# bronemos/view-fusion

Measured on AMD Instinct MI355X. Metric: denoise_steps_per_sec, higher is better.
Workload: dtype f32; 1 GPU; small UNet 64x64 (33.9M params), B=16/GPU N=6 (S=96 views/GPU), training iteration fwd+bwd+Adam, linear T=2000 schedule; global_batch=16, views=6, parallelism=dp1, launch=HIP-graph replay of the whole iteration

## Files before the change

view_fusion_amd/csrc/conv.hip:

```cpp
#include "common.h"
#include "wgrad_reduce.h"
#include <cstring>
#include "conv1x1.h"
#include "any_geom.h"
#include <cstdlib>

namespace {

constexpr int TCO = 64;
constexpr int WGRAD_TARGET_WGS = 512;

template <int KS, int LOGW, int MODE, int TPIX = 128>
struct Geo {
    static constexpr int W = 1 << LOGW;
    static constexpr int H = W;
    static constexpr int HW = W * H;
    static constexpr int IM = HW >= TPIX ? 1 : TPIX / HW;
    static constexpr int TH = HW >= TPIX ? TPIX / W : H;
    static constexpr int TPI = HW >= TPIX ? HW / TPIX : 1;
    static constexpr int PAD = KS / 2;
    static constexpr int PH = MODE == 1 ? 2 * TH + 1 : (MODE == 4 ? TH + 1 : TH + 2 * PAD);
    static constexpr int PW = KS == 1 ? W : (MODE == 1 ? 2 * W + 4 : (MODE == 4 ? W + 4 : W + 8));
    static constexpr int CO = (KS == 1 || MODE == 4) ? 0 : 3;
    static constexpr int Q = (MODE == 1 ? 2 * W : W) / 4;
    static constexpr int PS = IM * PH * PW;
    static constexpr int SH = MODE == 1 ? 2 * H : (MODE == 2 ? H / 2 : H);
    static constexpr int SW = MODE == 1 ? 2 * W : (MODE == 2 ? W / 2 : W);
    static __host__ __device__ constexpr int pix_off(int p) {
        const int im = IM > 1 ? (p >> (2 * LOGW)) : 0;
        const int q = p & (HW - 1);
        const int r = IM > 1 ? (q >> LOGW) : (p >> LOGW);
        const int c = p & (W - 1);
        return MODE == 1 ? im * PH * PW + 2 * r * PW + 2 * c + CO : im * PH * PW + r * PW + c + CO;
    }
};

struct ConvArgs {
    const float* x;
    const float* w;
    const float* bias;
    const float* vbias;
    const float* res;
    float* y;
    int S, Cin, Cout, CinP, CoutP;
    int ksplit;
    float* ws;
    const float* x2;
    float* y2;
    int C1, C1o;
    const float* gn_gamma = nullptr;
    const float* gn_beta = nullptr;
    float* gn_out = nullptr;
    float* gn_stats = nullptr;
    int gn_groups = 0, gn_silu = 0, gn_store_y = 1;
    float gn_eps = 1e-5f;
};

template <class G, int MODE, bool SAFE = false>
__device__ __forceinline__ float4 load_patch4(const float* __restrict__ x, int S, int Cin, int s, int ci,
                                              int r0, int pr, int q) {
    float4 v = make_float4(0.f, 0.f, 0.f, 0.f);
    if (SAFE && MODE == 0 && G::PAD == 0)
        return *reinterpret_cast<const float4*>(x + ((size_t)s * Cin + ci) * (size_t)(G::SH * G::SW) + (r0 + pr) * G::SW + 4 * q);
    if (s >= S || ci >= Cin) return v;
    const size_t plane = ((size_t)s * Cin + ci) * (size_t)(G::SH * G::SW);
    if (MODE == 0) {
        const int gy = r0 + pr - G::PAD;
        if (gy >= 0 && gy < G::H) v = *reinterpret_cast<const float4*>(x + plane + gy * G::SW + 4 * q);
    } else if (MODE == 1) {
        const int gy = 2 * r0 + pr - 1;
        if (gy >= 0 && gy < G::SH) v = *reinterpret_cast<const float4*>(x + plane + gy * G::SW + 4 * q);
    } else if (MODE == 4) {
        const int gy = r0 + pr;
        if (gy < G::H) v = *reinterpret_cast<const float4*>(x + plane + gy * G::SW + 4 * q);
    } else {
        const int uy = r0 + pr - G::PAD;
        if (uy >= 0 && uy < G::H) {
            const float2 t = *reinterpret_cast<const float2*>(x + plane + (uy >> 1) * G::SW + 2 * q);
            v = make_float4(t.x, t.x, t.y, t.y);
        }
    }
    return v;
}

template <int KS, int LOGW, int MODE, int NPT, int NCO = 1, bool SAFE = false>
__global__ __launch_bounds__(256, (KS == 1 && NPT == 1 && NCO == 1) ? 5 : 1) void conv_mfma_kernel(ConvArgs a) {
    constexpr int TPIX = 64 * NPT;
    using G = Geo<KS, LOGW, MODE, TPIX>;
    constexpr int CK = KS == 3 ? 8 : 32;
    constexpr int NG = KS == 3 ? 9 : 4;
    constexpr int WROW = 12;
    constexpr int NW4 = NG * TCO * 2;
    constexpr int NX4 = CK * G::IM * G::PH * G::Q;

    constexpr int WLS = NG * TCO * WROW;
    __shared__ __attribute__((aligned(16))) float wl[NCO * WLS];
    __shared__ __attribute__((aligned(16))) float xl[CK * G::PS];

    const int tid = threadIdx.x, lane = tid & 63, wid = tid >> 6;
    const int cw = wid & 1, pw = wid >> 1;
    const int li = lane & 31, lh = lane >> 5;

    const int ncot1 = a.CoutP / TCO;
    const int ncot = (ncot1 + NCO - 1) / NCO;
    const unsigned logical0 = xcd_remap(blockIdx.x, gridDim.x);
    const int split = logical0 % a.ksplit;
    const unsigned logical = logical0 / a.ksplit;
    const int cot = logical % ncot;
    const int tile = logical / ncot;
    const int co0 = cot * NCO * TCO;
    const int nco_here = min(NCO, ncot1 - cot * NCO);
    const int nch = a.CinP / CK;
    const int cbeg = (split * nch / a.ksplit) * CK, cend = ((split + 1) * nch / a.ksplit) * CK;
    const int s0 = G::IM > 1 ? tile * G::IM : tile / G::TPI;
    const int r0 = G::IM > 1 ? 0 : (tile % G::TPI) * G::TH;

#ifdef VF_CONV_STAMPS
    long long st_[4] = {clock64(), 0, 0, 0}, rt_[2] = {wall_clock64(), 0};
#endif
    if (KS != 1)
        for (int i = tid; i < CK * G::PS; i += 256) xl[i] = 0.f;

    constexpr int NWF = NW4 / 256, NXF = NX4 / 256;
    constexpr bool WT = (NW4 % 256) != 0, XT = (NX4 % 256) != 0;
    static_assert(NCO == 1 || !WT, "multi-tile workgroups assume whole 256-wide weight passes");
    constexpr int PD = 1;
    float4 wreg[PD][NCO * (NWF > 0 ? NWF : 1)], xreg[PD][NXF > 0 ? NXF : 1];
    float4 wtail[PD], xtail[PD];
#pragma unroll
    for (int d = 0; d < PD; ++d) wtail[d] = xtail[d] = make_float4(0.f, 0.f, 0.f, 0.f);
    const size_t wtile = (size_t)(a.CinP / CK) * (NG * TCO * 8);
    const float* wsrc = a.w + (size_t)cot * NCO * wtile;
    auto load_w = [&](int e, int c0, int j = 0) -> float4 {
        return *reinterpret_cast<const float4*>(wsrc + (size_t)min(j, nco_here - 1) * wtile +
                                                (size_t)(c0 / CK) * (NG * TCO * 8) + 4 * e);
    };
    auto load_x = [&](int e, int c0) -> float4 {
        const int q = e % G::Q;
        const int t1 = e / G::Q;
        const int pr = t1 % G::PH;
        const int t2 = t1 / G::PH;
        const int im = t2 % G::IM, ci = t2 / G::IM;
        if (KS == 1 && a.x2) {
            const bool second = c0 >= a.C1;
            return load_patch4<G, MODE, SAFE>(second ? a.x2 : a.x, a.S, second ? a.Cin - a.C1 : a.C1, s0 + im,
                                              second ? c0 - a.C1 + ci : c0 + ci, r0, pr, q);
        }
        return load_patch4<G, MODE, SAFE>(a.x, a.S, a.Cin, s0 + im, c0 + ci, r0, pr, q);
    };
    auto store_x = [&](int e, const float4& v) {
        const int q = e % G::Q;
        const int t1 = e / G::Q;
        *reinterpret_cast<float4*>(xl + t1 * G::PW + 4 * q + ((KS == 1 || MODE == 4) ? 0 : 4)) = v;
    };
#define VF_LOAD_CHUNK(D_, C0)                                                         \
    {                                                                                 \
// ... 247 lines not shown

    f32x16 acc[NT];
#pragma unroll
    for (int t = 0; t < NT; ++t) acc[t] = (f32x16){0};

    const float* ab = dyl + (cw * 32 + li) * DYS + kq * 64 + 4 * lh;
    const float* bb = xl + (ciw * 32 + li) * PSO + G::pix_off(kq * 64 + 4 * lh);

    constexpr int NXF = NX4 / 256;
    constexpr bool XT = (NX4 % 256) != 0;
    constexpr bool PF = BIG;
    float4 dreg[ND4 / 256], xreg[NXF > 0 ? NXF : 1];
    float4 xtail = make_float4(0.f, 0.f, 0.f, 0.f);
    auto load_dy = [&](int e, int tile) -> float4 {
        const int s0 = G::IM > 1 ? tile * G::IM : tile / G::TPI;
        const int r0 = G::IM > 1 ? 0 : (tile % G::TPI) * G::TH;
        const int q = e & 31, co = e >> 5;
        const int p = 4 * q;
        const int s = G::IM > 1 ? s0 + (p >> (2 * LOGW)) : s0;
        const int pix = G::IM > 1 ? (p & (OHW - 1)) : r0 * G::W + p;
        float4 v = make_float4(0.f, 0.f, 0.f, 0.f);
        if (s < a.S && co0 + co < a.Cout)
            v = *reinterpret_cast<const float4*>(a.dy + ((size_t)s * a.Cout + co0 + co) * OHW + pix);
        return v;
    };
    auto load_x = [&](int e, int tile) -> float4 {
        const int s0 = G::IM > 1 ? tile * G::IM : tile / G::TPI;
        const int r0 = G::IM > 1 ? 0 : (tile % G::TPI) * G::TH;
        const int q = e % G::Q;
        const int t1 = e / G::Q;
        const int pr = t1 % G::PH;
        const int t2 = t1 / G::PH;
        const int im = t2 % G::IM, ci = t2 / G::IM;
        if (KS == 1 && a.x2) {
            const bool second = ci0 >= a.C1;
            return load_patch4<G, MODE>(second ? a.x2 : a.x, a.S, second ? a.Cin - a.C1 : a.C1, s0 + im,
                                        second ? ci0 - a.C1 + ci : ci0 + ci, r0, pr, q);
        }
        return load_patch4<G, MODE>(a.x, a.S, a.Cin, s0 + im, ci0 + ci, r0, pr, q);
    };
    auto store_x = [&](int e, const float4& v) {
        const int q = e % G::Q;
        const int t1 = e / G::Q;
        const int ci = t1 / (G::IM * G::PH), rest = t1 % (G::IM * G::PH);
        float* d = xl + ci * PSO + rest * G::PW + 4 * q + (KS == 1 ? 0 : 4);
        d[0] = v.x; d[1] = v.y; d[2] = v.z; d[3] = v.w;
    };
#define VF_WG_LOAD(TILE)                                                                    \
    {                                                                                       \
        _Pragma("unroll") for (int i = 0; i < ND4 / 256; ++i) dreg[i] = load_dy(tid + i * 256, (TILE)); \
        _Pragma("unroll") for (int i = 0; i < NXF; ++i) xreg[i] = load_x(tid + i * 256, (TILE));        \
        if (XT && tid + NXF * 256 < NX4) xtail = load_x(tid + NXF * 256, (TILE));            \
    }
#define VF_WG_STORE()                                                                       \
    {                                                                                       \
        _Pragma("unroll") for (int i = 0; i < ND4 / 256; ++i) {                              \
            const int e = tid + i * 256;                                                    \
            *reinterpret_cast<float4*>(dyl + (e >> 5) * DYS + 4 * (e & 31)) = dreg[i];       \
        }                                                                                   \
        _Pragma("unroll") for (int i = 0; i < NXF; ++i) store_x(tid + i * 256, xreg[i]);     \
        if (XT && tid + NXF * 256 < NX4) store_x(tid + NXF * 256, xtail);                    \
    }

    if (PF && t_begin < t_end) VF_WG_LOAD(t_begin);
    for (int tile = t_begin; tile < t_end; ++tile) {
        __syncthreads();
        if (!PF) VF_WG_LOAD(tile);
        VF_WG_STORE();
        __syncthreads();
        if (PF && tile + 1 < t_end) VF_WG_LOAD(tile + 1);
        constexpr int NSTG = (BIG ? 16 : 8) * KS;
        auto frag_b = [&](int stg, int kw, int e) -> float {
            const int grp = stg / KS, kh = stg % KS;
            const int d = G::pix_off(8 * grp) - G::pix_off(0);
            return bb[d + (MODE == 1 ? 2 * e : e) + kh * G::PW + kw];
        };
        float b_cur[KS][4];
#pragma unroll
        for (int kw = 0; kw < KS; ++kw)
#pragma unroll
            for (int e = 0; e < 4; ++e) b_cur[kw][e] = frag_b(0, kw, e);
        float4 a4 = *reinterpret_cast<const float4*>(ab);
#pragma unroll
        for (int stg = 0; stg < NSTG; ++stg) {
            float b_nxt[KS][4];
            float4 a_nxt = a4;
            if (stg + 1 < NSTG) {
#pragma unroll
                for (int kw = 0; kw < KS; ++kw)
#pragma unroll
                    for (int e = 0; e < 4; ++e) b_nxt[kw][e] = frag_b(stg + 1, kw, e);
                if ((stg + 1) % KS == 0) a_nxt = *reinterpret_cast<const float4*>(ab + 8 * ((stg + 1) / KS));
            }
            __builtin_amdgcn_sched_barrier(0);
            const float av[4] = {a4.x, a4.y, a4.z, a4.w};
#pragma unroll
            for (int e = 0; e < 4; ++e)
#pragma unroll
                for (int kw = 0; kw < KS; ++kw) {
                    const int tap = (stg % KS) * KS + kw;
                    acc[tap] = __builtin_amdgcn_mfma_f32_32x32x2f32(av[e], b_cur[kw][e], acc[tap], 0, 0, 0);
                }
            __builtin_amdgcn_sched_barrier(0);
            if (stg + 1 < NSTG) {
                a4 = a_nxt;
#pragma unroll
                for (int kw = 0; kw < KS; ++kw)
#pragma unroll
                    for (int e = 0; e < 4; ++e) b_cur[kw][e] = b_nxt[kw][e];
            }
        }
    }

#undef VF_WG_LOAD
#undef VF_WG_STORE
    constexpr int NTP = NT > 1 ? (NT + 1) / 2 : 1;
    static_assert(2 * NTP * 16 * 64 <= LDSF, "k-half reduce buffer does not fit");
#pragma unroll
    for (int t0 = 0; t0 < (BIG ? 0 : NT); t0 += NTP) {
        __syncthreads();
        if (kq == 1) {
#pragma unroll
            for (int t = t0; t < (t0 + NTP < NT ? t0 + NTP : NT); ++t)
#pragma unroll
                for (int r = 0; r < 16; ++r) lds[((cw * NTP + (t - t0)) * 16 + r) * 64 + lane] = acc[t][r];
        }
        __syncthreads();
        if (kq == 0) {
#pragma unroll
            for (int t = t0; t < (t0 + NTP < NT ? t0 + NTP : NT); ++t)
#pragma unroll
                for (int r = 0; r < 16; ++r) acc[t][r] += lds[((cw * NTP + (t - t0)) * 16 + r) * 64 + lane];
        }
    }
    if (kq != 0) return;
    const int slab = bz;
#pragma unroll
    for (int tap = 0; tap < NT; ++tap) {
#pragma unroll
        for (int r = 0; r < 16; ++r) {
            const int co = co0 + cw * 32 + (r & 3) + 8 * (r >> 2) + 4 * lh;
            const int ci = ci0 + ciw * 32 + li;
            if (ci < a.CinQ) a.ws[(((size_t)slab * NT + tap) * a.CoutP + co) * a.CinQ + ci] = acc[tap][r];
        }
    }
}

__global__ __launch_bounds__(256) void wgrad_reduce_kernel(const float* __restrict__ ws, float* __restrict__ dw,
                                                           int nslab, int NT, int Cout, int Cin, int CoutP,
                                                           int CinQ) {
    wgrad_reduce_body(ws, dw, nslab, NT, Cout, Cin, CoutP, CinQ, (int)blockIdx.x);
}

struct Wgrad1Args {
    const float* x;
    const float* x2;
    const float* dy;
    float* ws;
    int S, Cin, Cout, CoutP, CinQ, C1, HW;
    int nsteps, steps_per_slice;
};

template <int TM, int TN>
__global__ __launch_bounds__(256, 2) void conv1x1_wgrad_kernel(Wgrad1Args a) {
    constexpr int KP = 64, RS = KP + 4;
    constexpr int NI = TM / 64, NJ = TN / 64;
    constexpr int ND = TM * 16 / 256, NX = TN * 16 / 256;
    __shared__ __attribute__((aligned(16))) float Dl[TM * RS];
    __shared__ __attribute__((aligned(16))) float Xl[TN * RS];
    const int tid = threadIdx.x, lane = tid & 63, wid = tid >> 6;
    const int cw = wid & 1, ciw = wid >> 1, li = lane & 31, lh = lane >> 5;
    const unsigned lgc = xcd_remap(blockIdx.x + gridDim.x * (blockIdx.y + gridDim.y * blockIdx.z),
                                   gridDim.x * gridDim.y * gridDim.z);
    const int bx = lgc % gridDim.x, by = (lgc / gridDim.x) % gridDim.y, bz = lgc / (gridDim.x * gridDim.y);
    const int co0 = bx * TM, ci0 = by * TN;
    const int t_begin = bz * a.steps_per_slice;
    const int t_end = min(a.nsteps, t_begin + a.steps_per_slice);
    const int spv = a.HW / KP;

    const int srow = tid >> 4, sq = tid & 15;
    size_t doff[8], xoff[8];
    const float* xb[8];
#pragma unroll
    for (int i = 0; i < 8; ++i) {
        const int row = srow + 16 * i;
        doff[i] = (size_t)min(co0 + row, a.Cout - 1) * a.HW + 4 * sq;
        const int ci = min(ci0 + row, a.Cin - 1);
        const bool second = a.x2 && ci >= a.C1;
        xb[i] = second ? a.x2 : a.x;
        xoff[i] = (size_t)(second ? ci - a.C1 : ci) * a.HW + 4 * sq;
    }
    const int xC = a.x2 ? a.C1 : a.Cin, x2C = a.Cin - a.C1;
    float4 dr0, dr1, dr2, dr3, dr4, dr5, dr6, dr7, xr0, xr1, xr2, xr3, xr4, xr5, xr6, xr7;
    dr0 = dr1 = dr2 = dr3 = dr4 = dr5 = dr6 = dr7 = xr0 = xr1 = xr2 = xr3 = xr4 = xr5 = xr6 = xr7 =
        make_float4(0.f, 0.f, 0.f, 0.f);
#define VF_W1_LD(I, T_)                                                                                   \
    {                                                                                                     \
        const int sv = (T_) / spv, p0 = ((T_) % spv) * KP;                                                 \
        if constexpr ((I) < ND)                                                                           \
            dr##I = *reinterpret_cast<const float4*>(a.dy + (size_t)sv * a.Cout * a.HW + doff[I] + p0);    \
        if constexpr ((I) < NX)                                                                           \
            xr##I = *reinterpret_cast<const float4*>(xb[I] + (size_t)sv * (xb[I] == a.x ? xC : x2C) * a.HW + xoff[I] + p0); \
    }
#define VF_W1_ST(I)                                                                                       \
    {                                                                                                     \
        if constexpr ((I) < ND) *reinterpret_cast<float4*>(Dl + (srow + 16 * (I)) * RS + 4 * sq) = dr##I;   \
        if constexpr ((I) < NX) *reinterpret_cast<float4*>(Xl + (srow + 16 * (I)) * RS + 4 * sq) = xr##I;   \
    }
#define VF_W1_LOAD(T_) { VF_W1_LD(0, T_) VF_W1_LD(1, T_) VF_W1_LD(2, T_) VF_W1_LD(3, T_) VF_W1_LD(4, T_) VF_W1_LD(5, T_) VF_W1_LD(6, T_) VF_W1_LD(7, T_) }
#define VF_W1_STORE() { VF_W1_ST(0) VF_W1_ST(1) VF_W1_ST(2) VF_W1_ST(3) VF_W1_ST(4) VF_W1_ST(5) VF_W1_ST(6) VF_W1_ST(7) }

    f32x16 acc[NI][NJ];
#pragma unroll
    for (int i = 0; i < NI; ++i)
#pragma unroll
        for (int j = 0; j < NJ; ++j) acc[i][j] = (f32x16){0};
    const float* ab = Dl + (cw * (TM / 2) + li) * RS + 4 * lh;
    const float* bb = Xl + (ciw * (TN / 2) + li) * RS + 4 * lh;

    if (t_begin < t_end) {
        VF_W1_LOAD(t_begin);
        for (int t = t_begin; t < t_end; ++t) {
            __syncthreads();
            VF_W1_STORE();
            __syncthreads();
            VF_W1_LOAD(min(t + 1, t_end - 1));
            float4 fa[NI], fb[NJ];
#pragma unroll
            for (int i = 0; i < NI; ++i) fa[i] = *reinterpret_cast<const float4*>(ab + 32 * i * RS);
#pragma unroll
            for (int j = 0; j < NJ; ++j) fb[j] = *reinterpret_cast<const float4*>(bb + 32 * j * RS);
#pragma unroll
            for (int g = 0; g < KP / 8; ++g) {
                float4 na[NI], nb[NJ];
#pragma unroll
                for (int i = 0; i < NI; ++i) na[i] = fa[i];
#pragma unroll
                for (int j = 0; j < NJ; ++j) nb[j] = fb[j];
                if (g + 1 < KP / 8) {
#pragma unroll
                    for (int i = 0; i < NI; ++i) na[i] = *reinterpret_cast<const float4*>(ab + 32 * i * RS + 8 * (g + 1));
#pragma unroll
                    for (int j = 0; j < NJ; ++j) nb[j] = *reinterpret_cast<const float4*>(bb + 32 * j * RS + 8 * (g + 1));
                }
                __builtin_amdgcn_sched_barrier(0);
#pragma unroll
                for (int i = 0; i < NI; ++i)
#pragma unroll
                    for (int j = 0; j < NJ; ++j) {
                        acc[i][j] = __builtin_amdgcn_mfma_f32_32x32x2f32(fa[i].x, fb[j].x, acc[i][j], 0, 0, 0);
                        acc[i][j] = __builtin_amdgcn_mfma_f32_32x32x2f32(fa[i].y, fb[j].y, acc[i][j], 0, 0, 0);
                        acc[i][j] = __builtin_amdgcn_mfma_f32_32x32x2f32(fa[i].z, fb[j].z, acc[i][j], 0, 0, 0);
                        acc[i][j] = __builtin_amdgcn_mfma_f32_32x32x2f32(fa[i].w, fb[j].w, acc[i][j], 0, 0, 0);
                    }
                __builtin_amdgcn_sched_barrier(0);
#pragma unroll
                for (int i = 0; i < NI; ++i) fa[i] = na[i];
#pragma unroll
                for (int j = 0; j < NJ; ++j) fb[j] = nb[j];
            }
        }
    }
#undef VF_W1_LD
#undef VF_W1_ST
#undef VF_W1_LOAD
#undef VF_W1_STORE
    float* sb = a.ws + (size_t)bz * a.CoutP * a.CinQ;
#pragma unroll
    for (int i = 0; i < NI; ++i)
#pragma unroll
        for (int j = 0; j < NJ; ++j) {
            const int ci = ci0 + ciw * (TN / 2) + j * 32 + li;
#pragma unroll
            for (int r = 0; r < 16; ++r) {
                const int co = co0 + cw * (TM / 2) + i * 32 + (r & 3) + 8 * (r >> 2) + 4 * lh;
                sb[(size_t)co * a.CinQ + ci] = acc[i][j][r];
            }
        }
}

__device__ __forceinline__ void pack_one(const float* __restrict__ w, float* __restrict__ wf,
                                         float* __restrict__ wb, int Cout, int Cin, int KS, size_t nf, size_t nb,
                                         size_t idx) {
    const int NT = KS * KS, CK = KS == 3 ? 8 : 32, NG = KS == 3 ? 9 : 4;
    const bool bwd = idx >= nf;
    if (bwd) {
        idx -= nf;
        if (idx >= nb || !wb) return;
    }
    const int M = bwd ? Cin : Cout, K = bwd ? Cout : Cin;
    const int nchunk = (K + CK - 1) / CK;
    const int k8 = idx & 7;
    const int m = (idx >> 3) & 63;
    size_t t = idx >> 9;
    const int g = t % NG;
    t /= NG;
    const int chunk = t % nchunk;
    const int mt = t / nchunk;
    const int mm = mt * 64 + m;
    const int kk = chunk * CK + (KS == 3 ? k8 : g * 8 + k8);
    const int tap = KS == 3 ? (bwd ? NT - 1 - g : g) : 0;
    float v = 0.f;
    if (mm < M && kk < K) {
        const int co = bwd ? kk : mm, ci = bwd ? mm : kk;
        v = w[((size_t)co * Cin + ci) * NT + tap];
    }
    (bwd ? wb : wf)[idx] = v;
}

__global__ void pack_weights_kernel(const float* __restrict__ w, float* __restrict__ wf, float* __restrict__ wb,
                                    int Cout, int Cin, int KS, size_t nf, size_t nb) {
    pack_one(w, wf, wb, Cout, Cin, KS, nf, nb, (size_t)blockIdx.x * blockDim.x + threadIdx.x);
}

struct PackDesc {
    const float* w;
    float* wf;
    float* wb;
    long long Cout, Cin, KS, nf, nb, first_block;
};
__global__ void pack_weights_multi_kernel(const PackDesc* __restrict__ desc, int nlayers) {
    int lo = 0, hi = nlayers;
    while (hi - lo > 1) {
        const int mid = (lo + hi) >> 1;
        if (desc[mid].first_block <= (long long)blockIdx.x) lo = mid; else hi = mid;
    }
    const PackDesc d = desc[lo];
    const size_t idx = ((size_t)blockIdx.x - (size_t)d.first_block) * blockDim.x + threadIdx.x;
    pack_one(d.w, d.wf, d.wb, (int)d.Cout, (int)d.Cin, (int)d.KS, (size_t)d.nf, (size_t)d.nb, idx);
}

__global__ void sumpool2_kernel(const float* __restrict__ x, float* __restrict__ y, size_t n_out, int Wo) {
    const size_t i = (size_t)blockIdx.x * blockDim.x + threadIdx.x;
    if (i >= n_out) return;
    const size_t row = i / Wo;
    const int w = i - row * Wo;
    const float* p = x + row * 2 * (2 * Wo) + 2 * w;
    y[i] = (p[0] + p[1]) + (p[2 * Wo] + p[2 * Wo + 1]);
}

__global__ void conv_splitk_reduce_kernel(const float4* __restrict__ ws, const float* __restrict__ bias,
                                          const float* __restrict__ vbias, const float4* __restrict__ res,
                                          float4* __restrict__ y, int ksplit, size_t n4, int HW4, int Cout) {
    const size_t i = (size_t)blockIdx.x * blockDim.x + threadIdx.x;
    if (i >= n4) return;
    const size_t sc = i / HW4;
    float b = 0.f;
    if (bias) b += bias[sc % Cout];
    if (vbias) b += vbias[sc];
    float4 r = make_float4(0.f, 0.f, 0.f, 0.f);
    if (res) r = res[i];
    float4 v = make_float4(0.f, 0.f, 0.f, 0.f);
    for (int k0 = 0; k0 < ksplit; k0 += 8) {
        float4 t[8];
#pragma unroll
        for (int j = 0; j < 8; ++j) t[j] = ws[(size_t)min(k0 + j, ksplit - 1) * n4 + i];
#pragma unroll
        for (int j = 0; j < 8; ++j) {
            if (k0 + j < ksplit) { v.x += t[j].x; v.y += t[j].y; v.z += t[j].z; v.w += t[j].w; }
        }
    }
    y[i] = make_float4(v.x + r.x + b, v.y + r.y + b, v.z + r.z + b, v.w + r.w + b);
}

template <int NV, int NT>
__global__ __launch_bounds__(NT) void conv_splitk_reduce_gn_kernel(const float4* __restrict__ ws, const float* __restrict__ bias,
                                                                    const float* __restrict__ vbias,
                                                                    const float4* __restrict__ res, float4* __restrict__ y,
                                                                    const float* __restrict__ gamma,
                                                                    const float* __restrict__ beta, float4* __restrict__ a_out,
                                                                    int ksplit, size_t n4_total, int hw4sh, int Cout, int cpg,
                                                                    float eps, int silu) {
    __shared__ float red[NT / 64];
    constexpr int KB = NV >= 8 ? 1 : 8 / NV;
    const int G = Cout / cpg;
    const int sg = blockIdx.x, s = sg / G, g = sg - s * G;
    const int n4 = cpg << hw4sh;
    const size_t base4 = ((size_t)s * Cout + (size_t)g * cpg) << hw4sh;
    float4 v[NV];
    size_t gi[NV];
#pragma unroll
    for (int i = 0; i < NV; ++i) {
        v[i] = make_float4(0.f, 0.f, 0.f, 0.f);
        gi[i] = base4 + min((int)threadIdx.x + i * NT, n4 - 1);
    }
    for (int k0 = 0; k0 < ksplit; k0 += KB) {
        float4 t[KB][NV];
#pragma unroll
        for (int kk = 0; kk < KB; ++kk)
#pragma unroll
            for (int i = 0; i < NV; ++i) t[kk][i] = ws[(size_t)min(k0 + kk, ksplit - 1) * n4_total + gi[i]];
#pragma unroll
        for (int kk = 0; kk < KB; ++kk)
            if (k0 + kk < ksplit) {
#pragma unroll
                for (int i = 0; i < NV; ++i) { v[i].x += t[kk][i].x; v[i].y += t[kk][i].y; v[i].z += t[kk][i].z; v[i].w += t[kk][i].w; }
            }
    }
    float gam[NV], bet[NV];
    float sum = 0.f;
#pragma unroll
    for (int i = 0; i < NV; ++i) {
        const int idx = min((int)threadIdx.x + i * NT, n4 - 1);
        const int c = g * cpg + (idx >> hw4sh);
        float b = 0.f;
        if (bias) b += bias[c];
        if (vbias) b += vbias[(size_t)s * Cout + c];
        float4 r = make_float4(0.f, 0.f, 0.f, 0.f);
        if (res) r = res[gi[i]];
        v[i] = make_float4(v[i].x + r.x + b, v[i].y + r.y + b, v[i].z + r.z + b, v[i].w + r.w + b);
        gam[i] = gamma[c];
        bet[i] = beta[c];
        const bool ok = (int)threadIdx.x + i * NT < n4;
        if (y && ok) y[gi[i]] = v[i];
        if (!ok) v[i] = make_float4(0.f, 0.f, 0.f, 0.f);
        sum += (v[i].x + v[i].y) + (v[i].z + v[i].w);
    }
    const float inv_n = 1.0f / (float)(n4 * 4);
    const float mean = block_sum<NT>(sum, red) * inv_n;
    float sq = 0.f;
#pragma unroll
    for (int i = 0; i < NV; ++i) {
        const float a = v[i].x - mean, b = v[i].y - mean, c = v[i].z - mean, d = v[i].w - mean;
        const float q = (a * a + b * b) + (c * c + d * d);
        sq += (int)threadIdx.x + i * NT < n4 ? q : 0.f;
    }
    const float var = block_sum<NT>(sq, red) * inv_n;
    const float rstd = 1.0f / sqrtf(var + eps);
#pragma unroll
    for (int i = 0; i < NV; ++i) {
        if ((int)threadIdx.x + i * NT < n4) {
            const float ga = gam[i] * rstd;
// ... 238 lines not shown
    hipLaunchKernelGGL(pack_weights_kernel, dim3((unsigned)((n + 255) / 256)), dim3(256), 0, (hipStream_t)stream,
                       w_oihw, w_fwd, w_bwd, Cout, Cin, KS, nf, nb);
    VF_RETURN_LAST_ERROR();
}

int vf_conv_pack_weights_multi(const void* desc, int nlayers, long total_blocks, void* stream) {
    if (nlayers <= 0 || total_blocks <= 0) return 0;
    hipLaunchKernelGGL(pack_weights_multi_kernel, dim3((unsigned)total_blocks), dim3(256), 0, (hipStream_t)stream,
                       (const PackDesc*)desc, nlayers);
    VF_RETURN_LAST_ERROR();
}

struct GnFuse {
    const float* gamma;
    const float* beta;
    float* out;
    float* stats;
    int groups, silu, store_y;
    float eps;
};

static int conv_fwd_impl(const float* x, const float* x2, int C1, const float* w_packed, const float* bias,
                         const float* view_bias, const float* residual, float* y, float* y2, int C1o, float* ws,
                         long ws_floats, int S, int Cin, int Cout, int H, int W, int KS, int mode, void* stream,
                         const GnFuse* gn = nullptr) {
    if (S <= 0) return 0;
    const int lw = ilog2_exact(W);
    if (!conv_fwd_args_ok(Cin, Cout, KS, mode, x2 != nullptr, C1, y2 != nullptr, C1o, gn != nullptr, gn ? gn->groups : 0))
        return (int)hipErrorInvalidValue;
    const ConvFwdPlan p = conv_fwd_plan(S, Cin, Cout, H, W, KS, mode, x2 != nullptr, C1, y2 != nullptr, C1o, gn != nullptr,
                                        gn ? gn->groups : 0, ws != nullptr, ws_floats);
    if (p.route == ROUTE_ANY) {
        const int e = vfi_conv_any_fwd(x, x2, C1, w_packed, bias, view_bias, residual, y, y2, C1o, ws, ws_floats, S, Cin, Cout,
                                       H, W, KS, mode, (hipStream_t)stream);
        if (e || !gn) return e;
        return vf_gn_fwd(y, gn->gamma, gn->beta, gn->out, gn->stats, gn->stats + (size_t)S * gn->groups, S, Cout, H * W,
                         gn->groups, gn->eps, gn->silu, stream);
    }
    ConvArgs a;
    a.x = x; a.w = w_packed; a.bias = bias; a.vbias = view_bias; a.res = residual; a.y = y;
    a.x2 = x2; a.C1 = C1; a.y2 = y2; a.C1o = C1o;
    if (y2) ws = nullptr;
    a.S = S; a.Cin = Cin; a.Cout = Cout;
    a.CinP = round_up(Cin, KS == 3 ? 8 : 32);
    a.CoutP = round_up(Cout, TCO);
    a.ksplit = 1;
    a.ws = ws;
    if (gn) {
        a.gn_gamma = gn->gamma; a.gn_beta = gn->beta; a.gn_out = gn->out; a.gn_stats = gn->stats;
        a.gn_groups = gn->groups; a.gn_silu = gn->silu; a.gn_store_y = gn->store_y; a.gn_eps = gn->eps;
    }
    hipStream_t st = (hipStream_t)stream;
    if (p.route == ROUTE_1X1_64 || p.route == ROUTE_1X1_128) {
        C11Args c = conv1x1_shape(S, Cin, Cout, H, W, C1, C1o);
        c.x = x; c.x2 = x2; c.w = w_packed; c.bias = bias; c.vbias = view_bias; c.res = residual; c.y = y; c.y2 = y2;
        return vfi_conv1x1_launch(c, st);
    }
#define VF_CASE(KS_, LW_, M_) \
    if (KS == KS_ && lw == LW_ && mode == M_) return launch_conv<KS_, LW_, M_>(a, st, p);
    VF_CASE(3, 3, 0) VF_CASE(3, 4, 0) VF_CASE(3, 5, 0) VF_CASE(3, 6, 0) VF_CASE(3, 7, 0)
    VF_CASE(3, 3, 1) VF_CASE(3, 4, 1) VF_CASE(3, 5, 1) VF_CASE(3, 6, 1)
    VF_CASE(3, 4, 2) VF_CASE(3, 5, 2) VF_CASE(3, 6, 2) VF_CASE(3, 7, 2)
    VF_CASE(3, 3, 4) VF_CASE(3, 4, 4) VF_CASE(3, 5, 4) VF_CASE(3, 6, 4)
    VF_CASE(1, 3, 0) VF_CASE(1, 4, 0) VF_CASE(1, 5, 0) VF_CASE(1, 6, 0) VF_CASE(1, 7, 0)
#undef VF_CASE
    return (int)hipErrorInvalidValue;
}

int vf_conv_fwd(const float* x, const float* w_packed, const float* bias, const float* view_bias,
                const float* residual, float* y, float* ws, long ws_floats, int S, int Cin, int Cout, int H,
                int W, int KS, int mode, void* stream) {
    return conv_fwd_impl(x, nullptr, Cin, w_packed, bias, view_bias, residual, y, nullptr, Cout, ws, ws_floats, S, Cin,
                         Cout, H, W, KS, mode, stream);
}

int vf_conv_fwd_gn(const float* x, const float* w_packed, const float* bias, const float* view_bias, const float* residual,
                   float* y, int store_y, const float* gn_gamma, const float* gn_beta, float* a_out, float* gn_stats,
                   int groups, float eps, int silu, float* ws, long ws_floats, int S, int Cin, int Cout, int H, int W,
                   int KS, int mode, void* stream) {
    GnFuse gn{gn_gamma, gn_beta, a_out, gn_stats, groups, silu, store_y, eps};
    return conv_fwd_impl(x, nullptr, Cin, w_packed, bias, view_bias, residual, y, nullptr, Cout, ws, ws_floats, S, Cin,
                         Cout, H, W, KS, mode, stream, &gn);
}

int vf_conv1x1_cat_fwd(const float* x1, const float* x2, int C1, const float* w_packed, const float* bias, float* y,
                       float* ws, long ws_floats, int S, int Cin, int Cout, int H, int W, void* stream) {
    return conv_fwd_impl(x1, x2, C1, w_packed, bias, nullptr, nullptr, y, nullptr, Cout, ws, ws_floats, S, Cin, Cout, H, W,
                         1, 0, stream);
}

int vf_conv1x1_cat_dgrad(const float* dy, const float* w_packed_bwd, float* dx1, float* dx2, int C1, int S, int Cin,
                         int Cout, int H, int W, void* stream) {
    return conv_fwd_impl(dy, nullptr, Cout, w_packed_bwd, nullptr, nullptr, nullptr, dx1, dx2, C1, nullptr, 0, S, Cout, Cin,
                         H, W, 1, 0, stream);
}

long vf_conv_fwd_ws_floats(int S, int Cin, int Cout, int H, int W, int KS) {
    if (!square_pow2(H, W)) return vfi_conv_any_fwd_ws_floats(S, Cin, Cout, H, W, KS);
    const long tiles64 = ((long)S * H * W + 63) / 64;
    const long nblk_min = ((long)S * H * W + 127) / 128 * (round_up(Cout, TCO) / TCO);
    (void)tiles64;
    const int nch = round_up(Cin, KS == 3 ? 8 : 32) / (KS == 3 ? 8 : 32);
    const int ks = choose_ksplit((int)nblk_min, nch);
    return ks > 1 ? (long)ks * S * Cout * H * W : 0;
}

int vf_conv_fwd_plan(int S, int Cin, int Cout, int H, int W, int KS, int mode, int C1, int C1o, int gn_groups, int has_ws,
                     long ws_floats, int* out) {
    if (!out || S <= 0 || Cin <= 0 || Cout <= 0 || H <= 0 || W <= 0) return (int)hipErrorInvalidValue;
    const bool cat = C1 > 0 && C1 < Cin, split = C1o > 0 && C1o < Cout, gn = gn_groups > 0;
    if (!conv_fwd_args_ok(Cin, Cout, KS, mode, cat, C1, split, C1o, gn, gn_groups)) return (int)hipErrorInvalidValue;
    if (mode != 0 && mode != 1 && mode != 2 && mode != 4) return (int)hipErrorInvalidValue;
    if (!fwd_specialised(KS, H, W, mode) && mode == 2 && ((H & 1) || (W & 1))) return (int)hipErrorInvalidValue;
    const ConvFwdPlan p = conv_fwd_plan(S, Cin, Cout, H, W, KS, mode, cat, C1, split, C1o, gn, gn_groups, has_ws != 0,
                                        ws_floats);
    const int v[8] = {p.route, p.npt, p.nblk, p.ks, p.safe, p.reduce, p.nv, p.nt};
    memcpy(out, v, sizeof v);
    return 0;
}

long vf_conv_wgrad_ws_floats(int S, int Cin, int Cout, int H, int W, int KS) {
    if (!square_pow2(H, W)) return vfi_conv_any_wgrad_ws_floats(S, Cin, Cout, H, W, KS);
    if (KS == 1) {
        const int tm = wgrad1_tile(Cout), tn = wgrad1_tile(Cin);
        const long slab1 = (long)round_up(Cout, tm) * round_up(Cin, tn);
        long z1 = WGRAD_TARGET_WGS / ((round_up(Cout, tm) / tm) * (round_up(Cin, tn) / tn));
        const long nsteps = (long)S * (H * W / 64);
        if (z1 > nsteps / 4) z1 = nsteps / 4;
        if (z1 < 1) z1 = 1;
        return z1 * slab1;
    }
    const long slab = (long)KS * KS * round_up(Cout, TCO) * round_up(Cin, 32);
    const int nco = round_up(Cout, TCO) / TCO, nci = round_up(Cin, 32) / 32;
    long z = (WGRAD_TARGET_WGS + nco * nci - 1) / (nco * nci);
    long ntiles = ((long)S * H * W + 127) / 128;
    if (z > ntiles) z = ntiles;
    if (z < 1) z = 1;
    return z * slab;
}

static int conv_wgrad_impl(const float* x, const float* x2, int C1, const float* dy, float* dw, float* ws,
                           long ws_floats, int S, int Cin, int Cout, int H, int W, int KS, int mode, void* stream,
                           long long* desc = nullptr, int* nblocks = nullptr) {
    if (desc) *nblocks = 0;
    if (S <= 0) return 0;
    const int lw = ilog2_exact(W);
    if (KS != 1 && KS != 3) return (int)hipErrorInvalidValue;
    if (KS == 1 && mode != 0) return (int)hipErrorInvalidValue;
    if (x2 && (KS != 1 || C1 <= 0 || C1 >= Cin || C1 % 64 != 0)) return (int)hipErrorInvalidValue;
    if (!wgrad_specialised(KS, H, W, mode))
        return vfi_conv_any_wgrad(x, x2, C1, dy, dw, ws, ws_floats, S, Cin, Cout, H, W, KS, mode, (hipStream_t)stream, desc,
                                  nblocks);
    if (KS == 1) {
        Wgrad1Args g;
        g.x = x; g.x2 = x2; g.dy = dy; g.ws = ws; g.S = S; g.Cin = Cin; g.Cout = Cout; g.C1 = C1; g.HW = H * W;
        const int tm = wgrad1_tile(Cout), tn = wgrad1_tile(Cin);
        g.CoutP = round_up(Cout, tm); g.CinQ = round_up(Cin, tn);
        g.nsteps = S * (H * W / 64);
        const int nco = g.CoutP / tm, nci = g.CinQ / tn;
        const size_t slab = (size_t)g.CoutP * g.CinQ;
        int z = WGRAD_TARGET_WGS / (nco * nci);
        if (z > g.nsteps / 4) z = g.nsteps / 4;
        if (z < 1) z = 1;
        if ((size_t)ws_floats < slab) return (int)hipErrorInvalidValue;
        if ((size_t)z > (size_t)ws_floats / slab) z = (int)((size_t)ws_floats / slab);
        g.steps_per_slice = (g.nsteps + z - 1) / z;
        z = (g.nsteps + g.steps_per_slice - 1) / g.steps_per_slice;
        hipStream_t st1 = (hipStream_t)stream;
        const dim3 grid(nco, nci, z);
        if (tm == 128 && tn == 128) hipLaunchKernelGGL((conv1x1_wgrad_kernel<128, 128>), grid, dim3(256), 0, st1, g);
        else if (tm == 128) hipLaunchKernelGGL((conv1x1_wgrad_kernel<128, 64>), grid, dim3(256), 0, st1, g);
        else if (tn == 128) hipLaunchKernelGGL((conv1x1_wgrad_kernel<64, 128>), grid, dim3(256), 0, st1, g);
        else hipLaunchKernelGGL((conv1x1_wgrad_kernel<64, 64>), grid, dim3(256), 0, st1, g);
        const int total = Cout * Cin;
        if (desc) {
            *nblocks = wgrad_reduce_row(desc, ws, dw, z, 1, Cout, Cin, g.CoutP, g.CinQ);
            VF_RETURN_LAST_ERROR();
        }
        hipLaunchKernelGGL(wgrad_reduce_kernel, dim3((total + 63) / 64), dim3(256), 0, st1, ws, dw, z, 1, Cout, Cin,
                           g.CoutP, g.CinQ);
        VF_RETURN_LAST_ERROR();
    }
    WgradArgs a;
    a.x = x; a.x2 = x2; a.C1 = C1; a.dy = dy; a.ws = ws; a.S = S; a.Cin = Cin; a.Cout = Cout;
    a.CoutP = round_up(Cout, TCO);
    a.CinQ = round_up(Cin, 32);
    hipStream_t st = (hipStream_t)stream;
#define VF_CASE(KS_, LW_, M_) \
    if (KS == KS_ && lw == LW_ && mode == M_) return launch_wgrad<KS_, LW_, M_>(a, dw, (size_t)ws_floats, st, desc, nblocks);
    VF_CASE(3, 3, 0) VF_CASE(3, 4, 0) VF_CASE(3, 5, 0) VF_CASE(3, 6, 0) VF_CASE(3, 7, 0)
    VF_CASE(3, 3, 1) VF_CASE(3, 4, 1) VF_CASE(3, 5, 1) VF_CASE(3, 6, 1)
    VF_CASE(3, 4, 2) VF_CASE(3, 5, 2) VF_CASE(3, 6, 2) VF_CASE(3, 7, 2)
#undef VF_CASE
    return (int)hipErrorInvalidValue;
}

int vf_conv_wgrad(const float* x, const float* dy, float* dw, float* ws, long ws_floats, int S, int Cin,
                  int Cout, int H, int W, int KS, int mode, void* stream) {
    return conv_wgrad_impl(x, nullptr, Cin, dy, dw, ws, ws_floats, S, Cin, Cout, H, W, KS, mode, stream);
}

int vf_conv1x1_cat_wgrad(const float* x1, const float* x2, int C1, const float* dy, float* dw, float* ws,
                         long ws_floats, int S, int Cin, int Cout, int H, int W, void* stream) {
    return conv_wgrad_impl(x1, x2, C1, dy, dw, ws, ws_floats, S, Cin, Cout, H, W, 1, 0, stream);
}

int vf_conv_wgrad_main(const float* x, const float* dy, float* dw, float* ws, long ws_floats, int S, int Cin, int Cout,
                       int H, int W, int KS, int mode, long long* desc9, int* nblocks, void* stream) {
    if (!desc9 || !nblocks) return (int)hipErrorInvalidValue;
    return conv_wgrad_impl(x, nullptr, Cin, dy, dw, ws, ws_floats, S, Cin, Cout, H, W, KS, mode, stream, desc9, nblocks);
}

int vf_conv1x1_cat_wgrad_main(const float* x1, const float* x2, int C1, const float* dy, float* dw, float* ws,
                              long ws_floats, int S, int Cin, int Cout, int H, int W, long long* desc9, int* nblocks,
                              void* stream) {
    if (!desc9 || !nblocks) return (int)hipErrorInvalidValue;
    return conv_wgrad_impl(x1, x2, C1, dy, dw, ws, ws_floats, S, Cin, Cout, H, W, 1, 0, stream, desc9, nblocks);
}

int vf_sumpool2(const float* x, float* y, long n_out, int Wo, void* stream) {
    if (n_out <= 0) return 0;
    hipLaunchKernelGGL(sumpool2_kernel, dim3((unsigned)((n_out + 255) / 256)), dim3(256), 0, (hipStream_t)stream,
                       x, y, (size_t)n_out, Wo);
    VF_RETURN_LAST_ERROR();
}

}
```

Baseline: 3207 view denoise-steps/s (UNet fwd+bwd per stacked view, incl. compose/MSE/Adam).

## Rewrite 1x1 conv weight-grad kernel with double-buffered LDS and interleaved loads

Moves the 1x1 weight-gradient GEMM kernel into its own file and restructures its main loop. It now double-buffers LDS, uses a smaller K-step for large tiles, and interleaves global loads, LDS stores and fragment reads between individual MFMAs. Addressing switches to 32-bit offsets with incrementally advanced pointers. This replaces a loop that took two barriers per step; the aim is to hide memory latency behind MFMA work. In exchange it adds a size guard that rejects tensors whose per-view byte offset would overflow 32 bits, and more complex scheduling code.

Result: no change. 3222 view denoise-steps/s (UNet fwd+bwd per stacked view, incl. compose/MSE/Adam) (median of 6 runs) (+0.5%).

```diff
diff --git a/view_fusion_amd/csrc/conv.hip b/view_fusion_amd/csrc/conv.hip
--- a/view_fusion_amd/csrc/conv.hip
+++ b/view_fusion_amd/csrc/conv.hip
@@ -2,6 +2,7 @@
 #include "wgrad_reduce.h"
 #include <cstring>
 #include "conv1x1.h"
+#include "conv1x1_wgrad.h"
 #include "any_geom.h"
 #include <cstdlib>
 
@@ -555,132 +556,6 @@
     wgrad_reduce_body(ws, dw, nslab, NT, Cout, Cin, CoutP, CinQ, (int)blockIdx.x);
 }
 
-struct Wgrad1Args {
-    const float* x;
-    const float* x2;
-    const float* dy;
-    float* ws;
-    int S, Cin, Cout, CoutP, CinQ, C1, HW;
-    int nsteps, steps_per_slice;
-};
-
-template <int TM, int TN>
-__global__ __launch_bounds__(256, 2) void conv1x1_wgrad_kernel(Wgrad1Args a) {
-    constexpr int KP = 64, RS = KP + 4;
-    constexpr int NI = TM / 64, NJ = TN / 64;
-    constexpr int ND = TM * 16 / 256, NX = TN * 16 / 256;
-    __shared__ __attribute__((aligned(16))) float Dl[TM * RS];
-    __shared__ __attribute__((aligned(16))) float Xl[TN * RS];
-    const int tid = threadIdx.x, lane = tid & 63, wid = tid >> 6;
-    const int cw = wid & 1, ciw = wid >> 1, li = lane & 31, lh = lane >> 5;
-    const unsigned lgc = xcd_remap(blockIdx.x + gridDim.x * (blockIdx.y + gridDim.y * blockIdx.z),
-                                   gridDim.x * gridDim.y * gridDim.z);
-    const int bx = lgc % gridDim.x, by = (lgc / gridDim.x) % gridDim.y, bz = lgc / (gridDim.x * gridDim.y);
-    const int co0 = bx * TM, ci0 = by * TN;
-    const int t_begin = bz * a.steps_per_slice;
-    const int t_end = min(a.nsteps, t_begin + a.steps_per_slice);
-    const int spv = a.HW / KP;
-
-    const int srow = tid >> 4, sq = tid & 15;
-    size_t doff[8], xoff[8];
-    const float* xb[8];
-#pragma unroll
-    for (int i = 0; i < 8; ++i) {
-        const int row = srow + 16 * i;
-        doff[i] = (size_t)min(co0 + row, a.Cout - 1) * a.HW + 4 * sq;
-        const int ci = min(ci0 + row, a.Cin - 1);
-        const bool second = a.x2 && ci >= a.C1;
-        xb[i] = second ? a.x2 : a.x;
-        xoff[i] = (size_t)(second ? ci - a.C1 : ci) * a.HW + 4 * sq;
-    }
-    const int xC = a.x2 ? a.C1 : a.Cin, x2C = a.Cin - a.C1;
-    float4 dr0, dr1, dr2, dr3, dr4, dr5, dr6, dr7, xr0, xr1, xr2, xr3, xr4, xr5, xr6, xr7;
-    dr0 = dr1 = dr2 = dr3 = dr4 = dr5 = dr6 = dr7 = xr0 = xr1 = xr2 = xr3 = xr4 = xr5 = xr6 = xr7 =
-        make_float4(0.f, 0.f, 0.f, 0.f);
-#define VF_W1_LD(I, T_)                                                                                   \
-    {                                                                                                     \
-        const int sv = (T_) / spv, p0 = ((T_) % spv) * KP;                                                 \
-        if constexpr ((I) < ND)                                                                           \
-            dr##I = *reinterpret_cast<const float4*>(a.dy + (size_t)sv * a.Cout * a.HW + doff[I] + p0);    \
-        if constexpr ((I) < NX)                                                                           \
-            xr##I = *reinterpret_cast<const float4*>(xb[I] + (size_t)sv * (xb[I] == a.x ? xC : x2C) * a.HW + xoff[I] + p0); \
-    }
-#define VF_W1_ST(I)                                                                                       \
-    {                                                                                                     \
-        if constexpr ((I) < ND) *reinterpret_cast<float4*>(Dl + (srow + 16 * (I)) * RS + 4 * sq) = dr##I;   \
-        if constexpr ((I) < NX) *reinterpret_cast<float4*>(Xl + (srow + 16 * (I)) * RS + 4 * sq) = xr##I;   \
-    }
-#define VF_W1_LOAD(T_) { VF_W1_LD(0, T_) VF_W1_LD(1, T_) VF_W1_LD(2, T_) VF_W1_LD(3, T_) VF_W1_LD(4, T_) VF_W1_LD(5, T_) VF_W1_LD(6, T_) VF_W1_LD(7, T_) }
-#define VF_W1_STORE() { VF_W1_ST(0) VF_W1_ST(1) VF_W1_ST(2) VF_W1_ST(3) VF_W1_ST(4) VF_W1_ST(5) VF_W1_ST(6) VF_W1_ST(7) }
-
-    f32x16 acc[NI][NJ];
-#pragma unroll
-    for (int i = 0; i < NI; ++i)
-#pragma unroll
-        for (int j = 0; j < NJ; ++j) acc[i][j] = (f32x16){0};
-    const float* ab = Dl + (cw * (TM / 2) + li) * RS + 4 * lh;
-    const float* bb = Xl + (ciw * (TN / 2) + li) * RS + 4 * lh;
-
-    if (t_begin < t_end) {
-        VF_W1_LOAD(t_begin);
-        for (int t = t_begin; t < t_end; ++t) {
-            __syncthreads();
-            VF_W1_STORE();
-            __syncthreads();
-            VF_W1_LOAD(min(t + 1, t_end - 1));
-            float4 fa[NI], fb[NJ];
-#pragma unroll
-            for (int i = 0; i < NI; ++i) fa[i] = *reinterpret_cast<const float4*>(ab + 32 * i * RS);
-#pragma unroll
-            for (int j = 0; j < NJ; ++j) fb[j] = *reinterpret_cast<const float4*>(bb + 32 * j * RS);
-#pragma unroll
-            for (int g = 0; g < KP / 8; ++g) {
-                float4 na[NI], nb[NJ];
-#pragma unroll
-                for (int i = 0; i < NI; ++i) na[i] = fa[i];
-#pragma unroll
-                for (int j = 0; j < NJ; ++j) nb[j] = fb[j];
-                if (g + 1 < KP / 8) {
-#pragma unroll
-                    for (int i = 0; i < NI; ++i) na[i] = *reinterpret_cast<const float4*>(ab + 32 * i * RS + 8 * (g + 1));
-#pragma unroll
-                    for (int j = 0; j < NJ; ++j) nb[j] = *reinterpret_cast<const float4*>(bb + 32 * j * RS + 8 * (g + 1));
-                }
-                __builtin_amdgcn_sched_barrier(0);
-#pragma unroll
-                for (int i = 0; i < NI; ++i)
-#pragma unroll
-                    for (int j = 0; j < NJ; ++j) {
-                        acc[i][j] = __builtin_amdgcn_mfma_f32_32x32x2f32(fa[i].x, fb[j].x, acc[i][j], 0, 0, 0);
-                        acc[i][j] = __builtin_amdgcn_mfma_f32_32x32x2f32(fa[i].y, fb[j].y, acc[i][j], 0, 0, 0);
-                        acc[i][j] = __builtin_amdgcn_mfma_f32_32x32x2f32(fa[i].z, fb[j].z, acc[i][j], 0, 0, 0);
-                        acc[i][j] = __builtin_amdgcn_mfma_f32_32x32x2f32(fa[i].w, fb[j].w, acc[i][j], 0, 0, 0);
-                    }
-                __builtin_amdgcn_sched_barrier(0);
-#pragma unroll
-                for (int i = 0; i < NI; ++i) fa[i] = na[i];
-#pragma unroll
-                for (int j = 0; j < NJ; ++j) fb[j] = nb[j];
-            }
-        }
-    }
-#undef VF_W1_LD
-#undef VF_W1_ST
-#undef VF_W1_LOAD
-#undef VF_W1_STORE
-    float* sb = a.ws + (size_t)bz * a.CoutP * a.CinQ;
-#pragma unroll
-    for (int i = 0; i < NI; ++i)
-#pragma unroll
-        for (int j = 0; j < NJ; ++j) {
-            const int ci = ci0 + ciw * (TN / 2) + j * 32 + li;
-#pragma unroll
-            for (int r = 0; r < 16; ++r) {
-                const int co = co0 + cw * (TM / 2) + i * 32 + (r & 3) + 8 * (r >> 2) + 4 * lh;
-                sb[(size_t)co * a.CinQ + ci] = acc[i][j][r];
-            }
-        }
-}
 
 __device__ __forceinline__ void pack_one(const float* __restrict__ w, float* __restrict__ wf,
                                          float* __restrict__ wb, int Cout, int Cin, int KS, size_t nf, size_t nb,
@@ -1225,6 +1100,7 @@
         return vfi_conv_any_wgrad(x, x2, C1, dy, dw, ws, ws_floats, S, Cin, Cout, H, W, KS, mode, (hipStream_t)stream, desc,
                                   nblocks);
     if (KS == 1) {
+        if ((size_t)(Cin > Cout ? Cin : Cout) * H * W * 4 >= (1ull << 32)) return (int)hipErrorInvalidValue;
         Wgrad1Args g;
         g.x = x; g.x2 = x2; g.dy = dy; g.ws = ws; g.S = S; g.Cin = Cin; g.Cout = Cout; g.C1 = C1; g.HW = H * W;
         const int tm = wgrad1_tile(Cout), tn = wgrad1_tile(Cin);
@@ -1241,10 +1117,7 @@
         z = (g.nsteps + g.steps_per_slice - 1) / g.steps_per_slice;
         hipStream_t st1 = (hipStream_t)stream;
         const dim3 grid(nco, nci, z);
-        if (tm == 128 && tn == 128) hipLaunchKernelGGL((conv1x1_wgrad_kernel<128, 128>), grid, dim3(256), 0, st1, g);
-        else if (tm == 128) hipLaunchKernelGGL((conv1x1_wgrad_kernel<128, 64>), grid, dim3(256), 0, st1, g);
-        else if (tn == 128) hipLaunchKernelGGL((conv1x1_wgrad_kernel<64, 128>), grid, dim3(256), 0, st1, g);
-        else hipLaunchKernelGGL((conv1x1_wgrad_kernel<64, 64>), grid, dim3(256), 0, st1, g);
+        vfi_conv1x1_wgrad_launch(g, tm, tn, grid, st1);
         const int total = Cout * Cin;
         if (desc) {
             *nblocks = wgrad_reduce_row(desc, ws, dw, z, 1, Cout, Cin, g.CoutP, g.CinQ);
diff --git a/view_fusion_amd/csrc/conv1x1_wgrad.h b/view_fusion_amd/csrc/conv1x1_wgrad.h
--- /dev/null
+++ b/view_fusion_amd/csrc/conv1x1_wgrad.h
@@ -0,0 +1,13 @@
+#pragma once
+#include <hip/hip_runtime.h>
+
+struct Wgrad1Args {
+    const float* x;
+    const float* x2;
+    const float* dy;
+    float* ws;
+    int S, Cin, Cout, CoutP, CinQ, C1, HW;
+    int nsteps, steps_per_slice;
+};
+
+void vfi_conv1x1_wgrad_launch(const Wgrad1Args& g, int tm, int tn, dim3 grid, hipStream_t st);
diff --git a/view_fusion_amd/csrc/conv1x1_wgrad.hip b/view_fusion_amd/csrc/conv1x1_wgrad.hip
--- /dev/null
+++ b/view_fusion_amd/csrc/conv1x1_wgrad.hip
@@ -0,0 +1,184 @@
+#include "common.h"
+#include "conv1x1_wgrad.h"
+
+namespace {
+
+#define VF_G1 __attribute__((address_space(1)))
+
+template <int TM, int TN>
+__global__ __launch_bounds__(256, 2) void conv1x1_wgrad_kernel(Wgrad1Args a) {
+    constexpr int KP = TM + TN > 128 ? 32 : 64;
+    constexpr int RS = KP + 4;
+    constexpr int SPS = 64 / KP;
+    constexpr int NG = KP / 8;
+    constexpr int NI = TM / 64, NJ = TN / 64;
+    constexpr int TPR = KP / 4;
+    constexpr int RPP = 256 / TPR;
+    constexpr int ND = TM / RPP, NX = TN / RPP;
+    constexpr int NL = ND + NX;
+    constexpr int STG = (TM + TN) * RS;
+    static_assert(2 * 2 * STG * 4 <= 160 * 1024, "two stages of two workgroups must fit the CU's LDS");
+    static_assert(NI * NJ * 4 >= 3 && NL >= NG, "a group needs three MFMAs to hide its side work behind");
+    __shared__ __attribute__((aligned(16))) float L[2 * STG];
+    const int tid = threadIdx.x, lane = tid & 63;
+    const int wid = __builtin_amdgcn_readfirstlane(tid >> 6);
+    const int cw = wid & 1, ciw = wid >> 1, li = lane & 31, lh = lane >> 5;
+    const unsigned lgc = xcd_remap(blockIdx.x + gridDim.x * (blockIdx.y + gridDim.y * blockIdx.z),
+                                   gridDim.x * gridDim.y * gridDim.z);
+    const int bx = lgc % gridDim.x, by = (lgc / gridDim.x) % gridDim.y, bz = lgc / (gridDim.x * gridDim.y);
+    const int co0 = bx * TM, ci0 = by * TN;
+    const int t_begin = bz * a.steps_per_slice;
+    const int t_end = min(a.nsteps, t_begin + a.steps_per_slice);
+    const int n = (t_end - t_begin) * SPS;
+
+    f32x16 acc[NI][NJ];
+#pragma unroll
+    for (int i = 0; i < NI; ++i)
+#pragma unroll
+        for (int j = 0; j < NJ; ++j) acc[i][j] = (f32x16){0};
+
+    if (n > 0) {
+        const int srow = tid / TPR, sq = tid % TPR;
+        unsigned dvo[ND], xvo[NX];
+#pragma unroll
+        for (int i = 0; i < ND; ++i)
+            dvo[i] = 4u * (unsigned)(min(co0 + srow + RPP * i, a.Cout - 1) * a.HW + 4 * sq);
+#pragma unroll
+        for (int i = 0; i < NX; ++i) {
+            const int ci = min(ci0 + srow + RPP * i, a.Cin - 1);
+            const bool second = a.x2 && ci >= a.C1;
+            xvo[i] = 4u * (unsigned)((second ? ci - a.C1 : ci) * a.HW + 4 * sq);
+        }
+        const int spv = a.HW / KP;
+        int ql = t_begin * SPS;
+        const int qlast = ql + n - 1;
+        const int sv = ql / spv;
+        int p0 = (ql - sv * spv) * KP;
+        const char* dptr = reinterpret_cast<const char*>(a.dy) + 4 * ((size_t)sv * a.Cout * a.HW + p0);
+        const size_t dwrap = 4 * ((size_t)(a.Cout - 1) * a.HW + KP);
+        const char* xptr[NJ];
+        size_t xwrap[NJ];
+#pragma unroll
+        for (int h = 0; h < NJ; ++h) {
+            const bool second = a.x2 && min(ci0 + 64 * h, a.Cin - 1) >= a.C1;
+            const int C = second ? a.Cin - a.C1 : (a.x2 ? a.C1 : a.Cin);
+            xptr[h] = reinterpret_cast<const char*>(second ? a.x2 : a.x) + 4 * ((size_t)sv * C * a.HW + p0);
+            xwrap[h] = 4 * ((size_t)(C - 1) * a.HW + KP);
+        }
+        auto advance = [&]() {
+            if (ql < qlast) {
+                ++ql;
+                p0 += KP;
+                const bool wrap = p0 == a.HW;
+                if (wrap) p0 = 0;
+                dptr += wrap ? dwrap : (size_t)(4 * KP);
+#pragma unroll
+                for (int h = 0; h < NJ; ++h) xptr[h] += wrap ? xwrap[h] : (size_t)(4 * KP);
+            }
+        };
+
+        f32x4 dr[2][ND], xr[2][NX];
+        auto load16 = [](const char* base, unsigned off) {
+            asm("" : "+s"(base), "+v"(off));
+            return *(const VF_G1 f32x4*)((const VF_G1 char*)base + off);
+        };
+        auto ld_ops = [&](int r, int lo, int hi) {
+#pragma unroll
+            for (int o = lo; o < hi; ++o) {
+                if (o < ND) dr[r][o] = load16(dptr, dvo[o]);
+                else xr[r][o - ND] = load16(xptr[(o - ND) * RPP / 64], xvo[o - ND]);
+            }
+        };
+        float* const sst = L + srow * RS + 4 * sq;
+        auto st_ops = [&](int r, int lo, int hi) {
+#pragma unroll
+            for (int o = lo; o < hi; ++o) {
+                if (o < ND) *reinterpret_cast<f32x4*>(sst + r * STG + RPP * o * RS) = dr[r][o];
+                else *reinterpret_cast<f32x4*>(sst + r * STG + (TM + RPP * (o - ND)) * RS) = xr[r][o - ND];
+            }
+        };
+
+        const float* const ab = L + (cw * (TM / 2) + li) * RS + 4 * lh;
+        const float* const bb = L + TM * RS + (ciw * (TN / 2) + li) * RS + 4 * lh;
+        f32x4 fa[NI], fb[NJ];
+#define VF_W1_FRAG(A, B, BUF, G)                                                                        \
+    {                                                                                                   \
+        _Pragma("unroll") for (int i = 0; i < NI; ++i)                                                  \
+            A[i] = *reinterpret_cast<const f32x4*>(ab + (BUF) * STG + 32 * i * RS + 8 * (G));           \
+        _Pragma("unroll") for (int j = 0; j < NJ; ++j)                                                  \
+            B[j] = *reinterpret_cast<const f32x4*>(bb + (BUF) * STG + 32 * j * RS + 8 * (G));           \
+    }
+
+        auto stage = [&](int P) {
+#pragma unroll
+            for (int g = 0; g < NG; ++g) {
+                f32x4 na[NI], nb[NJ];
+#pragma unroll
+                for (int i = 0; i < NI; ++i) na[i] = fa[i];
+#pragma unroll
+                for (int j = 0; j < NJ; ++j) nb[j] = fb[j];
+#pragma unroll
+                for (int e = 0; e < 4; ++e)
+#pragma unroll
+                    for (int i = 0; i < NI; ++i)
+#pragma unroll
+                        for (int j = 0; j < NJ; ++j) {
+                            const int m = (e * NI + i) * NJ + j;
+                            __builtin_amdgcn_sched_barrier(0);
+                            acc[i][j] = __builtin_amdgcn_mfma_f32_32x32x2f32(fa[i][e], fb[j][e], acc[i][j], 0, 0, 0);
+                            __builtin_amdgcn_sched_barrier(0);
+                            if (m == 0 && g + 1 < NG) VF_W1_FRAG(na, nb, P, g + 1);
+                            if (m == 1) st_ops(P ^ 1, g * NL / NG, (g + 1) * NL / NG);
+                            if (m == 2) ld_ops(P ^ 1, g * NL / NG, (g + 1) * NL / NG);
+                        }
+                __builtin_amdgcn_sched_barrier(0);
+#pragma unroll
+                for (int i = 0; i < NI; ++i) fa[i] = na[i];
+#pragma unroll
+                for (int j = 0; j < NJ; ++j) fb[j] = nb[j];
+            }
+            advance();
+            VF_LDS_BARRIER();
+            VF_W1_FRAG(fa, fb, P ^ 1, 0);
+        };
+
+        ld_ops(0, 0, NL);
+        advance();
+        ld_ops(1, 0, NL);
+        advance();
+        st_ops(0, 0, NL);
+        ld_ops(0, 0, NL);
+        advance();
+        VF_LDS_BARRIER();
+        VF_W1_FRAG(fa, fb, 0, 0);
+        int k = 0;
+        for (; k + 1 < n; k += 2) {
+            stage(0);
+            stage(1);
+        }
+        if (k < n) stage(0);
+#undef VF_W1_FRAG
+    }
+
+    float* sb = a.ws + (size_t)bz * a.CoutP * a.CinQ;
+#pragma unroll
+    for (int i = 0; i < NI; ++i)
+#pragma unroll
+        for (int j = 0; j < NJ; ++j) {
+            const int ci = ci0 + ciw * (TN / 2) + j * 32 + li;
+#pragma unroll
+            for (int r = 0; r < 16; ++r) {
+                const int co = co0 + cw * (TM / 2) + i * 32 + (r & 3) + 8 * (r >> 2) + 4 * lh;
+                sb[(size_t)co * a.CinQ + ci] = acc[i][j][r];
+            }
+        }
+}
+
+}
+
+void vfi_conv1x1_wgrad_launch(const Wgrad1Args& g, int tm, int tn, dim3 grid, hipStream_t st) {
+    if (tm == 128 && tn == 128) hipLaunchKernelGGL((conv1x1_wgrad_kernel<128, 128>), grid, dim3(256), 0, st, g);
+    else if (tm == 128) hipLaunchKernelGGL((conv1x1_wgrad_kernel<128, 64>), grid, dim3(256), 0, st, g);
+    else if (tn == 128) hipLaunchKernelGGL((conv1x1_wgrad_kernel<64, 128>), grid, dim3(256), 0, st, g);
+    else hipLaunchKernelGGL((conv1x1_wgrad_kernel<64, 64>), grid, dim3(256), 0, st, g);
+}
```
